# mokemokechicken/reversi-alpha-zero

Measured on NVIDIA H100. Metric: self_play_games_per_sec, higher is better.
Workload: dtype f16

## Files before the change

### reversi-alpha-zero_b200/csrc/rz_net_tc.cu

```cuda
#include <stdlib.h>
#include <mutex>
#include <type_traits>
#include "rz_bitboard.cuh"
#include "rz_net.cuh"
#include "rz_tc_common.cuh"

namespace rz {
namespace tc {

constexpr int kThreads = 384;
constexpr uint32_t kProducerRegs = 40, kMathRegs = 232;
constexpr int kMathThreads = 256;
constexpr uint32_t kActCg = 2896, kActSlot = 144;
constexpr uint32_t kActBytes = 32 * kActCg;
constexpr uint32_t kStageBytes = 32768, kStages = 3;
constexpr int kResAhead = 4;
constexpr uint32_t kA0Bytes = 8192, kW0Bytes = 16384;
constexpr uint32_t kOffAct = 0;
constexpr uint32_t kOffW = kOffAct + kActBytes;
constexpr uint32_t kOffA0 = kOffW + kStages * kStageBytes;
constexpr uint32_t kOffW0 = kOffA0 + kA0Bytes;
constexpr uint32_t kOffSS = kOffW0 + kW0Bytes;
constexpr uint32_t kOffHw = kOffSS + 2 * 2048;
constexpr uint32_t kOffBar = kOffHw + 768 * 4;
constexpr uint32_t kNumBars = 2 * kStages + 1;
constexpr uint32_t kSmemBytes = kOffBar + kNumBars * 8;
constexpr uint32_t kSmemAlloc = kSmemBytes + 128;
static_assert(kSmemAlloc <= 232448, "shared memory budget exceeded");
static_assert(kTowerResFloatsPerCta == (size_t)kMathThreads * 128, "residual scratch per CTA");

#ifdef RZ_TOWER_STAMPS
enum : int {
    kStTiles,
    kStTile,
    kStKLoop,
    kStFull,
    kStMma,
    kStEpiBar,
    kStEpi0,
    kStEpi1,
    kStEpi2,
    kStEpiLast,
    kStFeat,
    kStEmpty,
    kStCount
};
constexpr int kStMaxCtas = 1024;
__device__ unsigned long long g_tower_stamps[kStMaxCtas][kStCount];
__device__ __forceinline__ void stamp_add(int phase, uint32_t cycles) { atomicAdd(&g_tower_stamps[blockIdx.x][phase], (unsigned long long)cycles); }
#define RZ_STAMP(...) __VA_ARGS__
#else
#define RZ_STAMP(...)
#endif

template <int CL>
__global__ void __launch_bounds__(kThreads, 1) net_tower_kernel(const Params pp) {
    Params p = pp;
    if (p.n_dev) p.n = *p.n_dev;
    extern __shared__ uint8_t smem_raw[];
    const uint32_t base = (smem_u32(smem_raw) + 127u) & ~127u;
    uint8_t* sm = smem_raw + (base - smem_u32(smem_raw));
    const int warp = threadIdx.x >> 5, lane = threadIdx.x & 31;
    const uint32_t bar0 = base + kOffBar;
    auto bar_full = [&](uint32_t s) { return bar0 + s * 8; };
    auto bar_empty = [&](uint32_t s) { return bar0 + (kStages + s) * 8; };
    const uint32_t bar_w0 = bar0 + 2 * kStages * 8;
    const uint32_t ntiles = (p.n + 1) >> 1;
    const int L = p.n_layers;
    const uint32_t crank = CL > 1 ? cluster_ctarank() : 0u;
    const uint32_t cbase = blockIdx.x - crank;
    const uint32_t iters = cbase < ntiles ? (ntiles - cbase + gridDim.x - 1) / gridDim.x : 0u;

    for (uint32_t i = threadIdx.x * 16; i < kActBytes; i += kThreads * 16) *reinterpret_cast<uint4*>(sm + kOffAct + i) = make_uint4(0, 0, 0, 0);
    fence_proxy_async();
    for (uint32_t i = threadIdx.x; i < 768; i += kThreads)
        reinterpret_cast<float*>(sm + kOffHw)[i] = __ldg(i < 512 ? p.blob + p.off_policy_conv + i : p.blob + p.off_value_conv + (i - 512));
    if (threadIdx.x == 0) {
        for (uint32_t s = 0; s < kStages; ++s) { mbar_init(bar_full(s), 1); mbar_init(bar_empty(s), 8 * CL); }
        mbar_init(bar_w0, 1);
        asm volatile("fence.mbarrier_init.release.cluster;" ::: "memory");
    }
    __syncthreads();
    if (CL > 1) cluster_sync_all();

    if (warp >= 8) {
        asm volatile("setmaxnreg.dec.sync.aligned.u32 %0;" ::"n"(kProducerRegs));
        if (warp == 8 && lane == 0) {
            if (iters > 0) {
                mbar_expect_tx(bar_w0, kW0Bytes);
                bulk_g2s(base + kOffW0, p.w0, kW0Bytes, bar_w0);
            }
            uint32_t stage = 0, phase = 0;
            for (uint32_t it = 0; it < iters; ++it) {
                for (int l = 1; l < L; ++l) {
                    const uint8_t* src = reinterpret_cast<const uint8_t*>(p.w) + (size_t)(l - 1) * 36 * kStageBytes;
                    RZ_STAMP(uint32_t st_empty = 0;)
                    for (int s = 0; s < 36; ++s) {
                        RZ_STAMP(const uint32_t c0 = (uint32_t)clock();)
                        mbar_wait(bar_empty(stage), phase ^ 1);
                        RZ_STAMP(st_empty += (uint32_t)clock() - c0;)
                        mbar_expect_tx(bar_full(stage), kStageBytes);
                        if (CL == 1) {
                            bulk_g2s(base + kOffW + stage * kStageBytes, src + (size_t)s * kStageBytes, kStageBytes, bar_full(stage));
                        } else {
                            constexpr uint32_t kSlice = kStageBytes / CL;
                            bulk_g2s_mc(base + kOffW + stage * kStageBytes + crank * kSlice, src + (size_t)s * kStageBytes + crank * kSlice,
                                        kSlice, bar_full(stage), (uint16_t)((1u << CL) - 1u));
                        }
                        if (++stage == kStages) { stage = 0; phase ^= 1; }
                    }
                    RZ_STAMP(stamp_add(kStEmpty, st_empty);)
                }
            }
        }
    } else {
        asm volatile("setmaxnreg.inc.sync.aligned.u32 %0;" ::"n"(kMathRegs));
        const int et = threadIdx.x;
        const int wg = warp >> 2;
        const int r0 = wg * 64 + (warp & 3) * 16 + (lane >> 2);
        const int g0 = r0 >> 3, x = r0 & 7, y = g0 >> 1;
        const int cq = 2 * (lane & 3);
        const uint32_t act_row0 = base + kOffAct + (g0 + 2) * kActSlot + (x + 1) * 16 + cq * 2;
        const uint32_t act_row1 = act_row0 + kActSlot;
        const uint32_t a_wg = base + kOffAct + wg * 8 * kActSlot;
        float* ss_s = reinterpret_cast<float*>(sm + kOffSS);
        float4* res = reinterpret_cast<float4*>(p.res + (size_t)blockIdx.x * kTowerResFloatsPerCta) + et;
        const float* hw = reinterpret_cast<const float*>(sm + kOffHw);
        uint32_t stage = 0, phase = 0, ss_buf = 0;
        float d[128];
        ss_s[et] = __ldg(p.ss + et);
        ss_s[256 + et] = __ldg(p.ss + 256 + et);

        for (uint32_t it = 0; it < iters; ++it) {
            const uint32_t tile = blockIdx.x + it * gridDim.x;
            const uint32_t pos0 = tile * 2;
            RZ_STAMP(const uint32_t st_tile0 = (uint32_t)clock();)
            {
                const int m = et & 127, g = m >> 3, brd = g & 1;
                const bool valid = pos0 + brd < p.n;
                build_layer0_operand(sm + kOffA0, valid ? p.own[pos0 + brd] : 0, valid ? p.enemy[pos0 + brd] : 0, 2 * (et >> 7), g, m & 7,
                                     g >> 1);
                fence_proxy_async();
            }
            float hs[6];
            for (int l = 0; l < L; ++l) {
                const float* sc = ss_s + ss_buf * 512;
                const bool is_conv2 = l > 0 && (l & 1) == 0;
                float4 rb[kResAhead];
                RZ_STAMP(uint32_t st_c = (uint32_t)clock(), st_bar = 0, st_full = 0, st_mma = 0;)
                epi_bar();
                RZ_STAMP(st_bar += (uint32_t)clock() - st_c;)
                {
                    const size_t nl = l + 1 < L ? (size_t)l + 1 : 0;
                    const uint32_t dst = smem_u32(ss_s + (ss_buf ^ 1) * 512 + et);
                    cp_async_4(dst, p.ss + nl * 512 + et);
                    cp_async_4(dst + 1024, p.ss + nl * 512 + 256 + et);
                }
                RZ_STAMP(const uint32_t st_k0 = (uint32_t)clock();)
                acc_fence(d);
                if (l == 0) {
                    RZ_STAMP(st_c = (uint32_t)clock();)
                    mbar_wait(bar_w0, 0);
                    RZ_STAMP(st_full += (uint32_t)clock() - st_c;)
                    wgmma_fence();
#pragma unroll
                    for (uint32_t j = 0; j < 2; ++j)
                        wgmma_m64n256k16(d, smem_desc(base + kOffA0 + j * 2 * 2048 + wg * 1024, 2048, 128),
                                         smem_desc(base + kOffW0 + j * 2 * 4096, 4096, 128), j);
                    wgmma_commit();
                    RZ_STAMP(st_c = (uint32_t)clock();)
                    wgmma_wait<0>();
                    RZ_STAMP(st_mma += (uint32_t)clock() - st_c;)
                } else {
                    int prev = -1;
                    for (uint32_t tap = 0; tap < 9; ++tap) {
                        const uint32_t a_tap = a_wg + (2 * (tap / 3)) * kActSlot + (tap % 3) * 16;
                        for (uint32_t kb = 0; kb < 4; ++kb) {
                            RZ_STAMP(st_c = (uint32_t)clock();)
                            mbar_wait(bar_full(stage), phase);
                            RZ_STAMP(st_full += (uint32_t)clock() - st_c;)
                            const uint32_t b_st = base + kOffW + stage * kStageBytes;
                            wgmma_fence();
#pragma unroll
                            for (uint32_t j = 0; j < 4; ++j)
                                wgmma_m64n256k16(d, smem_desc(a_tap + (kb * 8 + 2 * j) * kActCg, kActCg, kActSlot),
                                                 smem_desc(b_st + 2 * j * 4096, 4096, 128), (tap | kb | j) != 0);
                            wgmma_commit();
                            RZ_STAMP(st_c = (uint32_t)clock();)
                            wgmma_wait<1>();
                            RZ_STAMP(st_mma += (uint32_t)clock() - st_c;)
                            if (prev >= 0 && lane == 0) {
                                mbar_arrive(bar_empty(prev));
                                if (CL > 1) mbar_arrive_cta(bar_empty(prev), crank ^ 1u);
                            }
                            prev = (int)stage;
                            if (++stage == kStages) { stage = 0; phase ^= 1; }
                        }
                    }
                    if (is_conv2) {
#pragma unroll
                        for (int i = 0; i < kResAhead; ++i) rb[i] = res[i * 256];
                    }
                    RZ_STAMP(st_c = (uint32_t)clock();)
                    wgmma_wait<0>();
                    RZ_STAMP(st_mma += (uint32_t)clock() - st_c;)
                    if (lane == 0) {
                        mbar_arrive(bar_empty(prev));
                        if (CL > 1) mbar_arrive_cta(bar_empty(prev), crank ^ 1u);
                    }
                }
                RZ_STAMP(const uint32_t st_k1 = (uint32_t)clock();)
                acc_fence(d);
                cp_async_wait_all();
                ss_buf ^= 1;
                const bool keep_res = l == 0 || is_conv2;
                const bool last = l == L - 1;
                RZ_STAMP(st_c = (uint32_t)clock();)
                if (!last) epi_bar();
                RZ_STAMP(const uint32_t st_e0 = (uint32_t)clock(); st_bar += st_e0 - st_c;)
                float* dbg0 = nullptr;
                float* dbg1 = nullptr;
                if (last && p.dbg_tower) {
                    if (pos0 < p.n) dbg0 = p.dbg_tower + ((size_t)pos0 * 64 + y * 8 + x) * 256;
                    if (pos0 + 1 < p.n) dbg1 = p.dbg_tower + ((size_t)(pos0 + 1) * 64 + y * 8 + x) * 256;
                }
                constexpr int kEpiRelu = 0, kEpiKeep = 1, kEpiLast = 2;
                auto epilogue = [&](auto conv2, auto kind) {
                    constexpr bool kConv2 = decltype(conv2)::value;
                    constexpr bool kKeep = decltype(kind)::value == kEpiKeep, kLast = decltype(kind)::value == kEpiLast;
                    if (kLast) {
#pragma unroll
                        for (int k = 0; k < 6; ++k) hs[k] = 0.f;
                    }
#pragma unroll
                for (int i = 0; i < 32; ++i) {
                    const int c = 8 * i + cq;
                    const float2 s = *reinterpret_cast<const float2*>(sc + c);
                    const float2 b = *reinterpret_cast<const float2*>(sc + 256 + c);
                    float v0 = fmaf(d[4 * i + 0], s.x, b.x), v1 = fmaf(d[4 * i + 1], s.y, b.y);
                    float v2 = fmaf(d[4 * i + 2], s.x, b.x), v3 = fmaf(d[4 * i + 3], s.y, b.y);
                    if (kConv2) {
                        const float4 r = rb[i % kResAhead];
                        if (i + kResAhead < 32) rb[i % kResAhead] = res[(i + kResAhead) * 256];
                        v0 += r.x; v1 += r.y; v2 += r.z; v3 += r.w;
                    }
                    if (kKeep || kLast) {
                        v0 = fmaxf(v0, 0.f); v1 = fmaxf(v1, 0.f); v2 = fmaxf(v2, 0.f); v3 = fmaxf(v3, 0.f);
                    }
                    if (!kLast) {
                        if (kKeep) res[i * 256] = make_float4(v0, v1, v2, v3);
                        const uint32_t h0 = pack_h2<!kKeep>(v0, v1);
                        const uint32_t h1 = pack_h2<!kKeep>(v2, v3);
                        const uint32_t off = (c >> 3) * kActCg;
                        asm volatile("st.shared.b32 [%0], %1;" ::"r"(act_row0 + off), "r"(h0) : "memory");
                        asm volatile("st.shared.b32 [%0], %1;" ::"r"(act_row1 + off), "r"(h1) : "memory");
                    } else {
                        const float4 w = *reinterpret_cast<const float4*>(hw + 2 * c);
                        const float2 wv = *reinterpret_cast<const float2*>(hw + 512 + c);
                        hs[0] = fmaf(v1, w.z, fmaf(v0, w.x, hs[0]));
                        hs[1] = fmaf(v1, w.w, fmaf(v0, w.y, hs[1]));
                        hs[2] = fmaf(v1, wv.y, fmaf(v0, wv.x, hs[2]));
                        hs[3] = fmaf(v3, w.z, fmaf(v2, w.x, hs[3]));
                        hs[4] = fmaf(v3, w.w, fmaf(v2, w.y, hs[4]));
                        hs[5] = fmaf(v3, wv.y, fmaf(v2, wv.x, hs[5]));
                        if (dbg0) *reinterpret_cast<float2*>(dbg0 + c) = make_float2(v0, v1);
                        if (dbg1) *reinterpret_cast<float2*>(dbg1 + c) = make_float2(v2, v3);
                    }
                }
                };
                using Conv2 = std::true_type;
                using NoConv2 = std::false_type;
                if (last) {
                    if (is_conv2) epilogue(Conv2(), std::integral_constant<int, kEpiLast>());
                    else epilogue(NoConv2(), std::integral_constant<int, kEpiLast>());
                } else if (is_conv2) {
                    epilogue(Conv2(), std::integral_constant<int, kEpiKeep>());
                } else if (keep_res) {
                    epilogue(NoConv2(), std::integral_constant<int, kEpiKeep>());
                } else {
                    epilogue(NoConv2(), std::integral_constant<int, kEpiRelu>());
                }
                if (!last) fence_proxy_async();
                RZ_STAMP(if (et == 0) {
                    stamp_add(kStKLoop, st_k1 - st_k0); stamp_add(kStFull, st_full); stamp_add(kStMma, st_mma); stamp_add(kStEpiBar, st_bar);
                    stamp_add(l == 0 ? kStEpi0 : last ? kStEpiLast : is_conv2 ? kStEpi2 : kStEpi1, (uint32_t)clock() - st_e0);
                })
            }
            RZ_STAMP(const uint32_t st_h0 = (uint32_t)clock();)
#pragma unroll
            for (int k = 0; k < 6; ++k) {
                hs[k] += __shfl_xor_sync(0xffffffffu, hs[k], 1);
                hs[k] += __shfl_xor_sync(0xffffffffu, hs[k], 2);
            }
            {
                const int q = lane & 3;
                if (q < 2 && pos0 + q < p.n) {
                    const float h0 = q ? hs[3] : hs[0], h1 = q ? hs[4] : hs[1], h2 = q ? hs[5] : hs[2];
                    store_head_features(p.feat + (size_t)(pos0 + q) * kHeadFeatures, p.ss + (size_t)L * 512, y * 8 + x, h0 + 0.f,
                                        h1 + 0.f, h2 + 0.f);
                }
            }
            RZ_STAMP(if (et == 0) {
                const uint32_t st_h1 = (uint32_t)clock();
                stamp_add(kStFeat, st_h1 - st_h0); stamp_add(kStTile, st_h1 - st_tile0); stamp_add(kStTiles, 1);
            })
        }
    }

    __syncthreads();
    if (CL > 1) cluster_sync_all();
}

__global__ void pack_w0_kernel(const float* __restrict__ k0, __half* __restrict__ out) {
    const int i = blockIdx.x * blockDim.x + threadIdx.x;
    if (i >= 4 * 256 * 8) return;
    const int j = i & 7, n = (i >> 3) & 255, kc = i >> 11, k = kc * 8 + j;
    out[i] = __float2half_rn(k < 18 ? k0[(size_t)k * 256 + n] : 0.f);
}
__global__ void pack_w_kernel(const float* __restrict__ blob, size_t off_res0, size_t stride, int n_layers, __half* __restrict__ out) {
    const size_t total = (size_t)n_layers * 36 * 8 * 256 * 8;
    for (size_t i = (size_t)blockIdx.x * blockDim.x + threadIdx.x; i < total; i += (size_t)gridDim.x * blockDim.x) {
        const int j = i & 7, n = (i >> 3) & 255, kc = (i >> 11) & 7;
        const size_t ls = i >> 14;
        const int s = (int)(ls % 36), l = (int)(ls / 36);
        const int tap = s >> 2, kb = s & 3, ci = kb * 64 + kc * 8 + j;
        out[i] = __float2half_rn(blob[off_res0 + (size_t)l * stride + ((size_t)tap * 256 + ci) * 256 + n]);
    }
}

}

int net_pack_tc(rz_net* net, cudaStream_t stream) {
    tc::pack_w0_kernel<<<(4 * 256 * 8 + 255) / 256, 256, 0, stream>>>(net->blob + net->off_conv0, net->tc_w0);
    if (net->cfg.res_blocks > 0)
        tc::pack_w_kernel<<<num_sms() * 8, 256, 0, stream>>>(net->blob, net->off_res0, net->res_stride_conv, 2 * net->cfg.res_blocks, net->tc_w);
    RZ_LAUNCH_CHECK();
    return RZ_OK;
}

static int g_cluster = 0;

int set_tower_cluster(int cluster) {
    RZ_REQUIRE(cluster == 1 || cluster == 2, "rz_net_set_tower_cluster: cluster must be 1 or 2");
    g_cluster = cluster;
    return RZ_OK;
}

int tower_cluster() {
    if (g_cluster == 0) {
        const char* cs = getenv("RZ_TOWER_CLUSTER");
        g_cluster = (cs && atoi(cs) == 1) ? 1 : 2;
    }
    return g_cluster;
}

int net_forward_tc(rz_net* net, const uint64_t* own, const uint64_t* enemy, float* policy, float* value, size_t n, cudaStream_t stream,
                   float* dbg_tower, const uint32_t* n_dev, float* dbg_logits, float* dbg_vlogit) {
    if (net->cfg.filters == 64 || net->cfg.filters == 128)
        return net_forward_tc_narrow(net, own, enemy, policy, value, n, stream, dbg_tower, n_dev, dbg_logits, dbg_vlogit);
    RZ_REQUIRE(net->cfg.filters == 256, "wgmma tower requires 64, 128 or 256 filters (got %d)", net->cfg.filters);
    RZ_REQUIRE(net->cfg.value_fc <= (int)tc::kTcMaxV, "wgmma tower supports value_fc_size <= %u", tc::kTcMaxV);
    RZ_REQUIRE(n < (1ull << 31), "batch too large");
    static int max_pairs = -1;
    if (max_pairs < 0) {
        RZ_CUDA_TRY(cudaFuncSetAttribute(tc::net_tower_kernel<1>, cudaFuncAttributeMaxDynamicSharedMemorySize, (int)tc::kSmemAlloc));
        RZ_CUDA_TRY(cudaFuncSetAttribute(tc::net_tower_kernel<2>, cudaFuncAttributeMaxDynamicSharedMemorySize, (int)tc::kSmemAlloc));
        cudaLaunchConfig_t cfg = {};
        cfg.gridDim = dim3((unsigned)num_sms() & ~1u); cfg.blockDim = dim3(tc::kThreads); cfg.dynamicSmemBytes = tc::kSmemAlloc;
        cudaLaunchAttribute attr[1];
        attr[0].id = cudaLaunchAttributeClusterDimension;
        attr[0].val.clusterDim.x = 2; attr[0].val.clusterDim.y = 1; attr[0].val.clusterDim.z = 1;
        cfg.attrs = attr; cfg.numAttrs = 1;
        RZ_CUDA_TRY(cudaOccupancyMaxActiveClusters(&max_pairs, tc::net_tower_kernel<2>, &cfg));
    }
    const int cluster = tower_cluster() == 2 && max_pairs >= 1 ? 2 : 1;
    tc::Params p;
    p.w0 = net->tc_w0; p.w = net->tc_w; p.ss = net->scale_shift; p.blob = net->blob;
    p.off_policy_conv = net->off_policy_conv; p.off_policy_fc_k = net->off_policy_fc_k; p.off_policy_fc_b = net->off_policy_fc_b;
    p.off_value_conv = net->off_value_conv; p.off_value_fc1_k = net->off_value_fc1_k; p.off_value_fc1_b = net->off_value_fc1_b;
    p.off_value_fc2_k = net->off_value_fc2_k; p.off_value_fc2_b = net->off_value_fc2_b;
    p.own = own; p.enemy = enemy; p.policy = policy; p.value = value; p.dbg_tower = dbg_tower;
    p.dbg_logits = dbg_logits; p.dbg_vlogit = dbg_vlogit;
    p.n = (uint32_t)n; p.n_dev = n_dev; p.n_layers = 1 + 2 * net->cfg.res_blocks; p.V = net->cfg.value_fc;
    p.res = net->res;
    std::lock_guard<std::mutex> lock(tower_mutex());
    RZ_TRY(head_features(net, n));
    p.feat = net->feat;
    RZ_CUDA_TRY(cudaStreamWaitEvent(stream, net->res_done, 0));
    const uint32_t ntiles = (uint32_t)((n + 1) / 2);
    uint32_t grid = ntiles < (uint32_t)num_sms() ? ntiles : (uint32_t)num_sms();
    if (cluster == 1) {
        tc::net_tower_kernel<1><<<grid, tc::kThreads, tc::kSmemAlloc, stream>>>(p);
    } else {
        grid = (grid + 1) & ~1u;
        if (grid > 2u * (uint32_t)max_pairs) grid = 2u * (uint32_t)max_pairs;
        cudaLaunchConfig_t cfg = {};
        cfg.gridDim = dim3(grid); cfg.blockDim = dim3(tc::kThreads); cfg.dynamicSmemBytes = tc::kSmemAlloc; cfg.stream = stream;
        cudaLaunchAttribute attr[1];
        attr[0].id = cudaLaunchAttributeClusterDimension;
        attr[0].val.clusterDim.x = 2; attr[0].val.clusterDim.y = 1; attr[0].val.clusterDim.z = 1;
        cfg.attrs = attr; cfg.numAttrs = 1;
        RZ_CUDA_TRY(cudaLaunchKernelEx(&cfg, tc::net_tower_kernel<2>, p));
    }
    RZ_LAUNCH_CHECK();
    RZ_TRY(net_heads(p, stream));
    RZ_CUDA_TRY(cudaEventRecord(net->res_done, stream));
    return RZ_OK;
}

}

#ifdef RZ_TOWER_STAMPS
extern "C" int rz_tower_stamps(unsigned long long* out, int n_ctas, int reset) {
    using namespace rz::tc;
    if (n_ctas < 0 || n_ctas > kStMaxCtas) return (int)cudaErrorInvalidValue;
    const size_t bytes = (size_t)n_ctas * kStCount * sizeof(unsigned long long);
    cudaError_t e = cudaDeviceSynchronize();
    if (e == cudaSuccess && out) e = cudaMemcpyFromSymbol(out, g_tower_stamps, bytes);
    if (e == cudaSuccess && reset) {
        void* dev = nullptr;
        e = cudaGetSymbolAddress(&dev, g_tower_stamps);
        if (e == cudaSuccess) e = cudaMemset(dev, 0, sizeof(g_tower_stamps));
        if (e == cudaSuccess) e = cudaDeviceSynchronize();
    }
    return (int)e;
}
extern "C" int rz_tower_stamp_count() { return rz::tc::kStCount; }
#endif
```

### reversi-alpha-zero_b200/csrc/rz_tc_common.cuh

```cuda
#pragma once
#include <cuda_fp16.h>
#include "rz_bitboard.cuh"
#include "rz_net.cuh"

namespace rz {
namespace tc {

__device__ __forceinline__ uint32_t smem_u32(const void* p) { return (uint32_t)__cvta_generic_to_shared(p); }

__device__ __forceinline__ void mbar_init(uint32_t bar, uint32_t count) {
    asm volatile("mbarrier.init.shared::cta.b64 [%0], %1;" ::"r"(bar), "r"(count) : "memory");
}
__device__ __forceinline__ void mbar_expect_tx(uint32_t bar, uint32_t bytes) {
    asm volatile("mbarrier.arrive.expect_tx.shared::cta.b64 _, [%0], %1;" ::"r"(bar), "r"(bytes) : "memory");
}
__device__ __forceinline__ void mbar_arrive(uint32_t bar) {
    asm volatile("mbarrier.arrive.shared::cta.b64 _, [%0];" ::"r"(bar) : "memory");
}
__device__ __forceinline__ void mbar_arrive_cta(uint32_t bar, uint32_t rank) {
    uint32_t remote;
    asm volatile("mapa.shared::cluster.u32 %0, %1, %2;" : "=r"(remote) : "r"(bar), "r"(rank));
    asm volatile("mbarrier.arrive.shared::cluster.b64 _, [%0];" ::"r"(remote) : "memory");
}
__device__ __forceinline__ void mbar_wait(uint32_t bar, uint32_t parity) {
    uint32_t ok = 0;
    long long t0 = 0;
    for (uint32_t spin = 0; !ok; ++spin) {
        asm volatile(
            "{\n\t.reg .pred p;\n\t"
            "mbarrier.try_wait.parity.shared::cta.b64 p, [%1], %2;\n\t"
            "selp.u32 %0, 1, 0, p;\n\t}"
            : "=r"(ok)
            : "r"(bar), "r"(parity)
            : "memory");
        if (!ok && (spin & 1023) == 1023) {
            const long long now = clock64();
            if (t0 == 0) t0 = now;
            else if (now - t0 > 8000000000LL) __trap();
        }
    }
}
__device__ __forceinline__ void bulk_g2s(uint32_t dst, const void* src, uint32_t bytes, uint32_t bar) {
    asm volatile("cp.async.bulk.shared::cluster.global.mbarrier::complete_tx::bytes [%0], [%1], %2, [%3];" ::"r"(dst), "l"(src),
                 "r"(bytes), "r"(bar)
                 : "memory");
}
__device__ __forceinline__ void bulk_g2s_mc(uint32_t dst, const void* src, uint32_t bytes, uint32_t bar, uint16_t mask) {
    asm volatile(
        "cp.async.bulk.shared::cluster.global.mbarrier::complete_tx::bytes.multicast::cluster [%0], [%1], %2, [%3], %4;" ::"r"(dst),
        "l"(src), "r"(bytes), "r"(bar), "h"(mask)
        : "memory");
}
__device__ __forceinline__ void cluster_sync_all() {
    asm volatile("barrier.cluster.arrive.release.aligned;\n\tbarrier.cluster.wait.acquire.aligned;" ::: "memory");
}
__device__ __forceinline__ uint32_t cluster_ctarank() {
    uint32_t r;
    asm volatile("mov.u32 %0, %%cluster_ctarank;" : "=r"(r));
    return r;
}
__device__ __forceinline__ void cp_async_4(uint32_t dst, const void* src) {
    asm volatile("cp.async.ca.shared.global [%0], [%1], 4;" ::"r"(dst), "l"(src) : "memory");
}
__device__ __forceinline__ void cp_async_wait_all() { asm volatile("cp.async.wait_all;" ::: "memory"); }
__device__ __forceinline__ void fence_proxy_async() { asm volatile("fence.proxy.async.shared::cta;" ::: "memory"); }
__device__ __forceinline__ void epi_bar() { asm volatile("bar.sync 1, 256;" ::: "memory"); }

__device__ __forceinline__ uint64_t smem_desc(uint32_t addr, uint32_t lbo, uint32_t sbo) {
    return (uint64_t)((addr >> 4) & 0x3FFF) | ((uint64_t)((lbo >> 4) & 0x3FFF) << 16) | ((uint64_t)((sbo >> 4) & 0x3FFF) << 32);
}
__device__ __forceinline__ void wgmma_fence() { asm volatile("wgmma.fence.sync.aligned;" ::: "memory"); }
__device__ __forceinline__ void wgmma_commit() { asm volatile("wgmma.commit_group.sync.aligned;" ::: "memory"); }
template <int N>
__device__ __forceinline__ void wgmma_wait() { asm volatile("wgmma.wait_group.sync.aligned %0;" ::"n"(N) : "memory"); }
__device__ __forceinline__ void acc_fence(float (&d)[128]) {
#pragma unroll
    for (int i = 0; i < 128; ++i) asm volatile("" : "+f"(d[i])::"memory");
}

#define RZ_D4(i) "+f"(d[i]), "+f"(d[i + 1]), "+f"(d[i + 2]), "+f"(d[i + 3])
#define RZ_D16(i) RZ_D4(i), RZ_D4(i + 4), RZ_D4(i + 8), RZ_D4(i + 12)
__device__ __forceinline__ void wgmma_m64n256k16(float (&d)[128], uint64_t adesc, uint64_t bdesc, uint32_t accumulate) {
    asm volatile(
        "{\n\t.reg .pred p;\n\t"
        "setp.ne.b32 p, %130, 0;\n\t"
        "wgmma.mma_async.sync.aligned.m64n256k16.f32.f16.f16 {"
        "%0, %1, %2, %3, %4, %5, %6, %7, %8, %9, %10, %11, %12, %13, %14, %15, "
        "%16, %17, %18, %19, %20, %21, %22, %23, %24, %25, %26, %27, %28, %29, %30, %31, "
        "%32, %33, %34, %35, %36, %37, %38, %39, %40, %41, %42, %43, %44, %45, %46, %47, "
        "%48, %49, %50, %51, %52, %53, %54, %55, %56, %57, %58, %59, %60, %61, %62, %63, "
        "%64, %65, %66, %67, %68, %69, %70, %71, %72, %73, %74, %75, %76, %77, %78, %79, "
        "%80, %81, %82, %83, %84, %85, %86, %87, %88, %89, %90, %91, %92, %93, %94, %95, "
        "%96, %97, %98, %99, %100, %101, %102, %103, %104, %105, %106, %107, %108, %109, %110, %111, "
        "%112, %113, %114, %115, %116, %117, %118, %119, %120, %121, %122, %123, %124, %125, %126, %127"
        "}, %128, %129, p, 1, 1, 0, 0;\n\t}"
        : RZ_D16(0), RZ_D16(16), RZ_D16(32), RZ_D16(48), RZ_D16(64), RZ_D16(80), RZ_D16(96), RZ_D16(112)
        : "l"(adesc), "l"(bdesc), "r"(accumulate)
        : "memory");
}
template <int O>
__device__ __forceinline__ void wgmma_m64n128k16(float (&d)[128], uint64_t adesc, uint64_t bdesc, uint32_t accumulate) {
    asm volatile(
        "{\n\t.reg .pred p;\n\t"
        "setp.ne.b32 p, %66, 0;\n\t"
        "wgmma.mma_async.sync.aligned.m64n128k16.f32.f16.f16 {"
        "%0, %1, %2, %3, %4, %5, %6, %7, %8, %9, %10, %11, %12, %13, %14, %15, "
        "%16, %17, %18, %19, %20, %21, %22, %23, %24, %25, %26, %27, %28, %29, %30, %31, "
        "%32, %33, %34, %35, %36, %37, %38, %39, %40, %41, %42, %43, %44, %45, %46, %47, "
        "%48, %49, %50, %51, %52, %53, %54, %55, %56, %57, %58, %59, %60, %61, %62, %63"
        "}, %64, %65, p, 1, 1, 0, 0;\n\t}"
        : RZ_D16(O), RZ_D16(O + 16), RZ_D16(O + 32), RZ_D16(O + 48)
        : "l"(adesc), "l"(bdesc), "r"(accumulate)
        : "memory");
}
template <int O>
__device__ __forceinline__ void wgmma_m64n64k16(float (&d)[128], uint64_t adesc, uint64_t bdesc, uint32_t accumulate) {
    asm volatile(
        "{\n\t.reg .pred p;\n\t"
        "setp.ne.b32 p, %34, 0;\n\t"
        "wgmma.mma_async.sync.aligned.m64n64k16.f32.f16.f16 {"
        "%0, %1, %2, %3, %4, %5, %6, %7, %8, %9, %10, %11, %12, %13, %14, %15, "
        "%16, %17, %18, %19, %20, %21, %22, %23, %24, %25, %26, %27, %28, %29, %30, %31"
        "}, %32, %33, p, 1, 1, 0, 0;\n\t}"
        : RZ_D16(O), RZ_D16(O + 16)
        : "l"(adesc), "l"(bdesc), "r"(accumulate)
        : "memory");
}
#undef RZ_D16
#undef RZ_D4

template <bool RELU>
__device__ __forceinline__ uint32_t pack_h2(float a, float b) {
    uint32_t d;
    if (RELU) asm("cvt.rn.relu.satfinite.f16x2.f32 %0, %1, %2;" : "=r"(d) : "f"(b), "f"(a));
    else      asm("cvt.rn.satfinite.f16x2.f32 %0, %1, %2;" : "=r"(d) : "f"(b), "f"(a));
    return d;
}

struct Params {
    const __half* w0;
    const __half* w;
    const float* ss;
    const float* blob;
    size_t off_policy_conv, off_policy_fc_k, off_policy_fc_b, off_value_conv, off_value_fc1_k, off_value_fc1_b, off_value_fc2_k,
        off_value_fc2_b;
    const u64* own;
    const u64* enemy;
    float* policy;
    float* value;
    float* res;
    float* feat;
    float* dbg_tower;
    float* dbg_logits;
    float* dbg_vlogit;
    uint32_t n;
    const uint32_t* n_dev;
    int n_layers;
    int V;
};

constexpr uint32_t kTcMaxV = 512;

__device__ __forceinline__ void build_layer0_operand(uint8_t* a0, u64 o, u64 e, int kc0, int g, int x, int y) {
#pragma unroll
    for (int kk = 0; kk < 2; ++kk) {
        const int kc = kc0 + kk;
        uint32_t w[4];
#pragma unroll
        for (int jp = 0; jp < 4; ++jp) {
            uint32_t packed = 0;
#pragma unroll
            for (int half = 0; half < 2; ++half) {
                const int k = kc * 8 + jp * 2 + half;
                uint32_t bit = 0;
                if (k < 18) {
                    const int tap = k >> 1, yy = y + tap / 3 - 1, xx = x + tap % 3 - 1;
                    if (yy >= 0 && yy < 8 && xx >= 0 && xx < 8) bit = (uint32_t)((((k & 1) ? e : o) >> (yy * 8 + xx)) & 1ULL);
                }
                packed |= (bit ? 0x3C00u : 0u) << (16 * half);
            }
            w[jp] = packed;
        }
        *reinterpret_cast<uint4*>(a0 + kc * 2048 + g * 128 + x * 16) = make_uint4(w[0], w[1], w[2], w[3]);
    }
}

__device__ __forceinline__ void store_head_features(float* f, const float* ssh, int pix, float a0, float a1, float av) {
    f[pix] = fmaxf(fmaf(a0, ssh[0], ssh[2]), 0.f);
    f[64 + pix] = fmaxf(fmaf(a1, ssh[1], ssh[3]), 0.f);
    f[128 + pix] = fmaxf(fmaf(av, ssh[4], ssh[5]), 0.f);
}

}

int net_heads(const tc::Params& p, cudaStream_t stream);

}
```

Measured before the change: 22.55.

## Use stmatrix for epilogue activation stores and interleave scale/shift in smem

Replaces the per-thread pairs of 32-bit shared stores of packed f16 activations with stmatrix.x4, issued every two column groups, using a per-lane row address derived from the fragment layout. Also reorders the per-channel scale and shift arrays in shared memory into an interleaved layout, so a single float4 load fetches both scale and bias, and updates the cp.async prefetch to match. The aim is to cut shared-memory store and load instruction counts in the epilogue. The cost is a denser address mapping that must exactly match the wgmma operand layout, and it holds an extra four registers.

```diff
diff --git a/reversi-alpha-zero_b200/csrc/rz_net_tc.cu b/reversi-alpha-zero_b200/csrc/rz_net_tc.cu
--- a/reversi-alpha-zero_b200/csrc/rz_net_tc.cu
+++ b/reversi-alpha-zero_b200/csrc/rz_net_tc.cu
@@ -120,16 +120,17 @@
         const int r0 = wg * 64 + (warp & 3) * 16 + (lane >> 2);
         const int g0 = r0 >> 3, x = r0 & 7, y = g0 >> 1;
         const int cq = 2 * (lane & 3);
-        const uint32_t act_row0 = base + kOffAct + (g0 + 2) * kActSlot + (x + 1) * 16 + cq * 2;
-        const uint32_t act_row1 = act_row0 + kActSlot;
+        const uint32_t stsm_row = base + kOffAct + (wg * 8 + 2 * (warp & 3) + 2 + ((lane >> 3) & 1)) * kActSlot +
+                                  ((lane & 7) + 1) * 16 + (lane >> 4) * kActCg;
         const uint32_t a_wg = base + kOffAct + wg * 8 * kActSlot;
         float* ss_s = reinterpret_cast<float*>(sm + kOffSS);
         float4* res = reinterpret_cast<float4*>(p.res + (size_t)blockIdx.x * kTowerResFloatsPerCta) + et;
         const float* hw = reinterpret_cast<const float*>(sm + kOffHw);
         uint32_t stage = 0, phase = 0, ss_buf = 0;
         float d[128];
-        ss_s[et] = __ldg(p.ss + et);
-        ss_s[256 + et] = __ldg(p.ss + 256 + et);
+        const int ss_et = (et >> 1) * 4 + (et & 1);
+        ss_s[ss_et] = __ldg(p.ss + et);
+        ss_s[ss_et + 2] = __ldg(p.ss + 256 + et);
 
         for (uint32_t it = 0; it < iters; ++it) {
             const uint32_t tile = blockIdx.x + it * gridDim.x;
@@ -152,9 +153,9 @@
                 RZ_STAMP(st_bar += (uint32_t)clock() - st_c;)
                 {
                     const size_t nl = l + 1 < L ? (size_t)l + 1 : 0;
-                    const uint32_t dst = smem_u32(ss_s + (ss_buf ^ 1) * 512 + et);
+                    const uint32_t dst = smem_u32(ss_s + (ss_buf ^ 1) * 512 + ss_et);
                     cp_async_4(dst, p.ss + nl * 512 + et);
-                    cp_async_4(dst + 1024, p.ss + nl * 512 + 256 + et);
+                    cp_async_4(dst + 8, p.ss + nl * 512 + 256 + et);
                 }
                 RZ_STAMP(const uint32_t st_k0 = (uint32_t)clock();)
                 acc_fence(d);
@@ -232,13 +233,13 @@
 #pragma unroll
                         for (int k = 0; k < 6; ++k) hs[k] = 0.f;
                     }
+                    uint32_t h[4];
 #pragma unroll
                 for (int i = 0; i < 32; ++i) {
                     const int c = 8 * i + cq;
-                    const float2 s = *reinterpret_cast<const float2*>(sc + c);
-                    const float2 b = *reinterpret_cast<const float2*>(sc + 256 + c);
-                    float v0 = fmaf(d[4 * i + 0], s.x, b.x), v1 = fmaf(d[4 * i + 1], s.y, b.y);
-                    float v2 = fmaf(d[4 * i + 2], s.x, b.x), v3 = fmaf(d[4 * i + 3], s.y, b.y);
+                    const float4 sb = *reinterpret_cast<const float4*>(sc + 2 * c);
+                    float v0 = fmaf(d[4 * i + 0], sb.x, sb.z), v1 = fmaf(d[4 * i + 1], sb.y, sb.w);
+                    float v2 = fmaf(d[4 * i + 2], sb.x, sb.z), v3 = fmaf(d[4 * i + 3], sb.y, sb.w);
                     if (kConv2) {
                         const float4 r = rb[i % kResAhead];
                         if (i + kResAhead < 32) rb[i % kResAhead] = res[(i + kResAhead) * 256];
@@ -249,11 +250,9 @@
                     }
                     if (!kLast) {
                         if (kKeep) res[i * 256] = make_float4(v0, v1, v2, v3);
-                        const uint32_t h0 = pack_h2<!kKeep>(v0, v1);
-                        const uint32_t h1 = pack_h2<!kKeep>(v2, v3);
-                        const uint32_t off = (c >> 3) * kActCg;
-                        asm volatile("st.shared.b32 [%0], %1;" ::"r"(act_row0 + off), "r"(h0) : "memory");
-                        asm volatile("st.shared.b32 [%0], %1;" ::"r"(act_row1 + off), "r"(h1) : "memory");
+                        h[2 * (i & 1)] = pack_h2<!kKeep>(v0, v1);
+                        h[2 * (i & 1) + 1] = pack_h2<!kKeep>(v2, v3);
+                        if (i & 1) stmatrix_x4(stsm_row + (i - 1) * kActCg, h[0], h[1], h[2], h[3]);
                     } else {
                         const float4 w = *reinterpret_cast<const float4*>(hw + 2 * c);
                         const float2 wv = *reinterpret_cast<const float2*>(hw + 512 + c);
diff --git a/reversi-alpha-zero_b200/csrc/rz_tc_common.cuh b/reversi-alpha-zero_b200/csrc/rz_tc_common.cuh
--- a/reversi-alpha-zero_b200/csrc/rz_tc_common.cuh
+++ b/reversi-alpha-zero_b200/csrc/rz_tc_common.cuh
@@ -63,6 +63,10 @@
     asm volatile("cp.async.ca.shared.global [%0], [%1], 4;" ::"r"(dst), "l"(src) : "memory");
 }
 __device__ __forceinline__ void cp_async_wait_all() { asm volatile("cp.async.wait_all;" ::: "memory"); }
+__device__ __forceinline__ void stmatrix_x4(uint32_t addr, uint32_t r0, uint32_t r1, uint32_t r2, uint32_t r3) {
+    asm volatile("stmatrix.sync.aligned.m8n8.x4.shared.b16 [%0], {%1, %2, %3, %4};" ::"r"(addr), "r"(r0), "r"(r1), "r"(r2), "r"(r3)
+                 : "memory");
+}
 __device__ __forceinline__ void fence_proxy_async() { asm volatile("fence.proxy.async.shared::cta;" ::: "memory"); }
 __device__ __forceinline__ void epi_bar() { asm volatile("bar.sync 1, 256;" ::: "memory"); }
 
```

New measurement: 22.58, median of 6. Within noise of the previous version (+0.1%).
